# cornell-zhang/HiSparse

Hardware: AMD Instinct MI355X
Metric: SpMV GBPS (8 B per non-zero per SpMV, sw/benchmark.cpp:312-346) (higher is better)
Workload: dtype u32 (Q8.24 fixed point, u64 row sums)

## Files before the change

hisparse_amd/csrc/hs_api.cpp:

```cpp
#include "hs_context.h"

#include <algorithm>
#include <cctype>
#include <cstdlib>
#include <cstring>
#include <mutex>
#include <new>

#include "gpu_tiles.h"

namespace {

thread_local std::string g_create_error;

const char* const kOptionKeys[] = {
    "STREAM_FORMAT", "COL_SLICES", "MAX_ROWS", "CROSS_PARTITIONS", "SPMM_VECTORS", "ROW_RUNS", "AUX_BITS", "XCD_AFFINITY", "STREAM_RESIDENT", "RETILE", "PLAN_DEBUG",
    "BITMAP_SKEW", "BITMAP_X_LDS", "BITMAP_BUILD", "WALK_LANES", "NO_MFMA_IMAGE", "MFMA_CHUNK", "LIGHT", "LIGHT_WGS", "SWEEP",
    "DELTA_DEAL", "POW2_SLICES", "SPMM_FUSED", "SPMM_MFMA", "SPMSPV", "SPMSPV_CROSSOVER", "ITERATE_GRAPH", "BATCH_GRAPH", "CARRY_COMBINE", "AUTOTUNE", "PLAN_CENSUS",
    "VALUE_MAP",
};

hisparse::dev::SpmvLaunch launch_args(const hs_context* c, const uint32_t* x, uint32_t* y, int32_t filter) {
    hisparse::dev::SpmvLaunch a = c->mat.launch;
    a.x = x;
    a.out = c->mat.col_slices > 1 ? c->carry.partial() : y;
    a.row_part_filter = filter;
    return a;
}

void partition_rows(const hs_context* c, uint32_t j, uint32_t& lo, uint32_t& hi) {
    const uint64_t a = uint64_t(j) * c->geom.logical_ob;
    const uint64_t b = std::min<uint64_t>(a + c->geom.logical_ob, c->mat.num_rows);
    lo = uint32_t(a);
    hi = uint32_t(b);
}

int step(hs_context* c, int32_t filter = -1, const Feedback* feedback = nullptr) { return enqueue(c, c->x_source(), c->y_target(), filter, nullptr, nullptr, feedback); }

}

int fail(hs_context* ctx, int code, const std::string& msg) {
    if (ctx) ctx->error = msg; else g_create_error = msg;
    return code;
}
int hip_fail(hs_context* ctx, hipError_t e, const char* what) {
    return fail(ctx, HS_ERR_HIP, std::string(what) + ": " + hipGetErrorString(e));
}

int settle(hs_context* c) {
    const hipError_t e = c->carry.settle(c->stream);
    return e == hipSuccess ? HS_OK : hip_fail(c, e, "combine_slices_kernel");
}

int enter(hs_context* ctx, unsigned need) {
    if (!ctx) return HS_ERR_BAD_ARG;
    if ((need & kMatrix) && !ctx->mat.loaded) return fail(ctx, HS_ERR_NOT_LOADED, "hs_load_matrix has not been called");
    if (need & kVector) {
        if (!ctx->vector_loaded && !ctx->x_bound) return fail(ctx, HS_ERR_NOT_LOADED, "hs_load_vector has not been called");
        if (!ctx->x_bound && ctx->x_len != ctx->mat.num_cols)
            return fail(ctx, HS_ERR_NOT_LOADED, "the loaded vector does not have this matrix's padded column count: call hs_load_vector again");
    }
    if ((need & kCsc) && !ctx->csc.indptr) return fail(ctx, HS_ERR_NOT_LOADED, "hs_load_matrix_csc has not been called");
    if ((need & kHostOnly) == kHostOnly) return HS_OK;
    HS_HIP(ctx, hipSetDevice(ctx->device));
    return (need & kNoSettle) ? HS_OK : settle(ctx);
}
int enter(hs_context* ctx, unsigned need, bool have_args) {
    if (!ctx || !have_args) return fail(ctx, HS_ERR_BAD_ARG, "null argument");
    return enter(ctx, need);
}

void drop_batch_graph(hs_context* c) {
    if (c->batch_exec) (void)hipGraphExecDestroy(c->batch_exec);
    if (c->batch_graph) (void)hipGraphDestroy(c->batch_graph);
    c->batch_exec = nullptr;
    c->batch_graph = nullptr;
    c->batch_steps = 0;
}

// ... 55 lines not shown
    int rc = HS_OK;
    for (int i = 0; i < warm && rc == HS_OK; ++i) rc = enqueue(c, x, y, -1, nullptr, nullptr);
    for (int rep = 0; rep < regions && rc == HS_OK; ++rep) {
        (void)hipEventRecord(t0.get(), c->stream);
        for (int i = 0; i < runs && rc == HS_OK; ++i) rc = enqueue(c, x, y, -1, nullptr, nullptr);
        if (rc == HS_OK) rc = settle(c);
        (void)hipEventRecord(t1.get(), c->stream);
        float ms = 0.0f;
        if (rc == HS_OK && hipEventSynchronize(t1.get()) == hipSuccess && hipEventElapsedTime(&ms, t0.get(), t1.get()) == hipSuccess) {
            const double one = double(ms) * 1000.0 / runs;
            *us = *us < 0.0 ? one : std::min(*us, one);
        }
    }
    if (rc != HS_OK) {
        c->carry.forget();
        *us = -1.0;
    }
    return rc;
}

extern "C" {

const char* hs_strerror(int code) {
    switch (code) {
        case HS_OK: return "ok";
        case HS_ERR_BAD_ARG: return "bad argument";
        case HS_ERR_NO_DEVICE: return "no usable gfx950 device";
        case HS_ERR_HIP: return "HIP runtime error";
        case HS_ERR_BAD_MATRIX: return "channel buffers are not a valid CPSR image";
        case HS_ERR_NOT_LOADED: return "matrix or vector not loaded";
        case HS_ERR_UNSUPPORTED: return "unsupported configuration";
        case HS_ERR_NO_MEMORY: return "out of memory";
        default: return "unknown error";
    }
}

const char* hs_last_error(const hs_context* ctx) { return ctx ? ctx->error.c_str() : g_create_error.c_str(); }

int hs_create(hs_context** out, int device_id, int impl, uint32_t ob_bank, uint32_t vb_bank) {
    if (!out) return fail(nullptr, HS_ERR_BAD_ARG, "null context pointer");
    *out = nullptr;
    if (!hisparse::impl_valid(impl)) return fail(nullptr, HS_ERR_BAD_ARG, "impl must be 0 (fixed), 1 (float_pob) or 2 (float_stall)");
    int count = 0;
    hipError_t e = hipGetDeviceCount(&count);
    if (e != hipSuccess || count <= 0) return fail(nullptr, HS_ERR_NO_DEVICE, "no HIP device visible (this library has no CPU fallback)");
    if (device_id < 0 || device_id >= count) return fail(nullptr, HS_ERR_BAD_ARG, "device_id out of range");
    hipDeviceProp_t prop;
    if ((e = hipGetDeviceProperties(&prop, device_id)) != hipSuccess) return hip_fail(nullptr, e, "hipGetDeviceProperties");
    if (std::strncmp(prop.gcnArchName, "gfx950", 6) != 0)
        return fail(nullptr, HS_ERR_NO_DEVICE, std::string("device is ") + prop.gcnArchName + ", this library carries gfx950 code only");
    hs_context* c = new (std::nothrow) hs_context;
    if (!c) return fail(nullptr, HS_ERR_NO_MEMORY, "out of memory");
    c->device = device_id;
    c->impl = impl;
    c->geom = hisparse::make_geometry(impl, ob_bank ? ob_bank : hisparse::impl_default_ob_bank(impl),
                                      vb_bank ? vb_bank : hisparse::impl_default_vb_bank(impl));
    c->compute_units = prop.multiProcessorCount;
    if (c->geom.logical_ob > 0xffffffffull || c->geom.logical_vb > 0xffffffffull || c->geom.logical_ob % c->geom.row_divisor != 0) {
        delete c;
        return fail(nullptr, HS_ERR_BAD_ARG, "ob_bank must make 128*ob_bank a multiple of 128*interleave; bank sizes must fit 32 bits");
    }
    if ((e = hipSetDevice(device_id)) != hipSuccess || (e = hipStreamCreateWithFlags(&c->own_stream, hipStreamNonBlocking)) != hipSuccess) {
        delete c;
        return hip_fail(nullptr, e, "hipSetDevice/hipStreamCreate");
    }
    c->stream = c->own_stream;
    if ((e = hisparse::dev::configure_spmv_kernels(hisparse::dev::kMaxLdsBytes)) != hipSuccess || (e = hisparse::dev::warm_gpu_tiler()) != hipSuccess) {
        (void)hipStreamDestroy(c->own_stream);
        delete c;
        return hip_fail(nullptr, e, "loading the gfx950 kernels");
    }
    static std::once_flag copy_paths;
    std::call_once(copy_paths, [c] {
        std::vector<uint8_t> host(4 << 20, 0);
        DeviceBuffer<uint8_t> dev;
        if (dev.alloc(host.size()) != hipSuccess) return;
        (void)hipMemcpy(dev.get(), host.data(), host.size(), hipMemcpyHostToDevice);
        (void)hipMemcpy(host.data(), dev.get(), host.size(), hipMemcpyDeviceToHost);
        (void)hipMemcpyAsync(dev.get(), host.data(), host.size(), hipMemcpyHostToDevice, c->own_stream);
        (void)hipMemcpyAsync(host.data(), dev.get(), host.size(), hipMemcpyDeviceToHost, c->own_stream);
        (void)hipStreamSynchronize(c->own_stream);
    });
    *out = c;
    return HS_OK;
}

int hs_destroy(hs_context* ctx) {
    if (!ctx) return HS_OK;
    (void)hipSetDevice(ctx->device);
    if (ctx->stream == ctx->own_stream) (void)hipStreamSynchronize(ctx->own_stream);
    else (void)hipDeviceSynchronize();
    free_matrix(ctx);
    ctx->csc = CscData();
    ctx->d_x.reset();
    if (ctx->own_stream) (void)hipStreamDestroy(ctx->own_stream);
    delete ctx;
    return HS_OK;
}

int hs_load_vector(hs_context* ctx, const void* packed_x, uint32_t num_cols) {
    if (!ctx || !packed_x) return fail(ctx, HS_ERR_BAD_ARG, "null argument");
    if (ctx->mat.loaded && num_cols != ctx->mat.num_cols) return fail(ctx, HS_ERR_BAD_ARG, "vector length must equal the padded column count");
    if (int rc = enter(ctx, kNoSettle)) return rc;
    if (num_cols > ctx->x_capacity) {
        HS_HIP(ctx, hipStreamSynchronize(ctx->stream));
        ctx->x_capacity = 0;
        HS_HIP(ctx, ctx->d_x.alloc(size_t(num_cols) * 4 + 64));
        ctx->x_capacity = num_cols;
    }
    HS_HIP(ctx, hipMemcpyAsync(ctx->d_x.get(), packed_x, size_t(num_cols) * 4, hipMemcpyHostToDevice, ctx->stream));
    HS_HIP(ctx, hipStreamSynchronize(ctx->stream));
    ctx->vector_loaded = true;
    ctx->x_len = num_cols;
    return HS_OK;
}

int hs_run(hs_context* ctx) {
    if (int rc = enter(ctx, kReady | kNoSettle)) return rc;
    return step(ctx);
}

int hs_run_batch(hs_context* ctx, uint32_t steps) {
    int rc = enter(ctx, kReady | kNoSettle | (steps ? 0u : kHostOnly));
    if (rc != HS_OK || steps == 0) return rc;
    const char* opt = ctx_option(ctx, "HISPARSE_BATCH_GRAPH");
    struct InBatch {
        hs_context* c;
        const bool own;
        explicit InBatch(hs_context* ctx) : c(ctx), own(ctx->stream_private()) { c->in_batch = true; }
        ~InBatch() { c->in_batch = false; }
        int settle() { return own ? HS_OK : ::settle(c); }
    } batch(ctx);
    if (!(opt && std::atoi(opt) != 0)) {
        for (uint32_t i = 0; i < steps; ++i)
            if ((rc = step(ctx)) != HS_OK) {
                (void)batch.settle();
                return rc;
            }
        return batch.settle();
    }
    if (const char* why = hisparse::dev::profiling_switch_error()) return fail(ctx, HS_ERR_BAD_ARG, why);
    if (!ctx->batch_exec || ctx->batch_steps != steps || ctx->batch_x != ctx->x_source() || ctx->batch_y != ctx->y_target() || ctx->batch_stream != ctx->stream) {
        drop_batch_graph(ctx);
        if ((rc = ::settle(ctx)) != HS_OK) return rc;
        hipError_t e = hipStreamBeginCapture(ctx->stream, hipStreamCaptureModeThreadLocal);
        if (e != hipSuccess) return hip_fail(ctx, e, "hipStreamBeginCapture (the legacy default stream cannot be captured)");
        for (uint32_t i = 0; i < steps && rc == HS_OK; ++i) rc = step(ctx);
        if (rc == HS_OK) rc = ::settle(ctx);
        e = hipStreamEndCapture(ctx->stream, &ctx->batch_graph);
        if (rc == HS_OK && (e != hipSuccess || !ctx->batch_graph)) rc = hip_fail(ctx, e, "hipStreamEndCapture");
        if (rc == HS_OK && (e = hipGraphInstantiate(&ctx->batch_exec, ctx->batch_graph, nullptr, nullptr, 0)) != hipSuccess) rc = hip_fail(ctx, e, "hipGraphInstantiate");
        if (rc != HS_OK) {
            ctx->carry.forget();
            drop_batch_graph(ctx);
            return rc;
        }
        ctx->batch_steps = steps;
        ctx->batch_x = ctx->x_source();
        ctx->batch_y = ctx->y_target();
        ctx->batch_stream = ctx->stream;
    }
    if ((rc = ::settle(ctx)) != HS_OK) return rc;
    HS_HIP(ctx, hipGraphLaunch(ctx->batch_exec, ctx->stream));
    return HS_OK;
}

int hs_run_partition(hs_context* ctx, uint32_t row_part_id, uint32_t part_len) {
    if (int rc = enter(ctx, kReady | kNoSettle)) return rc;
    if (row_part_id >= ctx->mat.row_parts) return fail(ctx, HS_ERR_BAD_ARG, "row_part_id out of range");
    uint32_t lo, hi;
    partition_rows(ctx, row_part_id, lo, hi);
    if (part_len != (hi - lo) / hisparse::NUM_HBM_CHANNELS)
        return fail(ctx, HS_ERR_BAD_ARG, "part_len must be the partition's rows / 16 (sw/benchmark.cpp:301-322): expected " +
                                             std::to_string((hi - lo) / hisparse::NUM_HBM_CHANNELS));
    return step(ctx, int32_t(row_part_id));
}

int hs_feedback(hs_context* ctx, uint32_t scale_word, uint32_t shift_word) {
    if (int rc = enter(ctx, kReady)) return rc;
    HS_HIP(ctx, hisparse::dev::launch_feedback(ctx->is_float(), ctx->y_target(), const_cast<uint32_t*>(ctx->x_source()),
                                               std::min(ctx->mat.num_rows, ctx->mat.num_cols), scale_word, shift_word, ctx->stream));
    return HS_OK;
}

int hs_iterate(hs_context* ctx, uint32_t iterations, uint32_t scale_word, uint32_t shift_word) {
    int rc = enter(ctx, kReady | (iterations ? 0u : kHostOnly));
    if (rc != HS_OK || iterations == 0) return rc;
    const Feedback feedback{scale_word, shift_word};
    auto one_iteration = [&]() -> int { return step(ctx, -1, &feedback); };
    const char* graph_env = ctx_option(ctx, "HISPARSE_ITERATE_GRAPH");
    const bool use_graph = graph_env && std::atoi(graph_env) != 0;
    const uint32_t chunk = use_graph ? std::min<uint32_t>(iterations, 32) : 1;
    uint32_t done = 0;
    hipGraph_t graph = nullptr;
    hipGraphExec_t exec = nullptr;
    if (chunk > 1 && hipStreamBeginCapture(ctx->stream, hipStreamCaptureModeThreadLocal) == hipSuccess) {
        for (uint32_t i = 0; i < chunk && rc == HS_OK; ++i) rc = one_iteration();
        const hipError_t end = hipStreamEndCapture(ctx->stream, &graph);
        if (rc == HS_OK && end == hipSuccess && graph && hipGraphInstantiate(&exec, graph, nullptr, nullptr, 0) == hipSuccess) {
            hipError_t e = hipSuccess;
            for (; done + chunk <= iterations && e == hipSuccess; done += chunk) e = hipGraphLaunch(exec, ctx->stream);
            (void)hipGraphExecDestroy(exec);
            (void)hipGraphDestroy(graph);
            if (e != hipSuccess) return fail(ctx, HS_ERR_HIP, std::string("hipGraphLaunch: ") + hipGetErrorString(e));
        } else {
            if (graph) (void)hipGraphDestroy(graph);
            (void)hipGetLastError();
            if (rc != HS_OK) return rc;
        }
    } else {
        (void)hipGetLastError();
    }
    for (; done < iterations; ++done)
        if ((rc = one_iteration()) != HS_OK) return rc;
    return HS_OK;
}

int hs_sync(hs_context* ctx) {
    if (int rc = enter(ctx, 0)) return rc;
    HS_HIP(ctx, hipStreamSynchronize(ctx->stream));
    return HS_OK;
}

int hs_read_result(hs_context* ctx, void* packed_y, uint32_t num_rows) {
    if (int rc = enter(ctx, kMatrix | kNoSettle, packed_y != nullptr)) return rc;
    if (num_rows != ctx->mat.num_rows) return fail(ctx, HS_ERR_BAD_ARG, "result length must equal the padded row count");
    if (int rc = settle(ctx)) return rc;
    HS_HIP(ctx, hipMemcpyAsync(packed_y, ctx->y_target(), size_t(num_rows) * 4, hipMemcpyDeviceToHost, ctx->stream));
    HS_HIP(ctx, hipStreamSynchronize(ctx->stream));
    return HS_OK;
}

int hs_set_option(hs_context* ctx, const char* key, const char* value) {
    if (int rc = enter(ctx, kHostOnly, key != nullptr)) return rc;
    std::string k(key);
    for (char& ch : k) ch = char(std::toupper(static_cast<unsigned char>(ch)));
    if (k.rfind("HISPARSE_", 0) == 0) k = k.substr(9);
    bool known = false;
    for (const char* name : kOptionKeys) known = known || k == name;
    if (k == "ABLATE" || k == "DEPTH" || k == "TIMELINE_OUT")
        return fail(ctx, HS_ERR_BAD_ARG, "'" + k + "' is a profiling switch of libhisparse_hip_prof.so (wrong results by design), not an option of this library");
    if (!known) return fail(ctx, HS_ERR_BAD_ARG, "unknown option '" + std::string(key) + "'");
    if (value && *value && k == "MFMA_CHUNK") {
        uint32_t chunk = 0;
        if (!hisparse::dev::detail::parse_mfma_chunk(value, chunk)) return fail(ctx, HS_ERR_BAD_ARG, hisparse::dev::detail::kBadMfmaChunk);
    }
    if (value && *value) ctx->options["HISPARSE_" + k] = value;
    else ctx->options.erase("HISPARSE_" + k);
    drop_batch_graph(ctx);
    return HS_OK;
}

int hs_set_stream(hs_context* ctx, void* hip_stream) {
    if (int rc = enter(ctx, 0)) return rc;
// ... 52 lines not shown
    if (num_words > ctx->mat.num_rows || (num_words & 3u)) return fail(ctx, HS_ERR_BAD_ARG, "num_words must be a multiple of 4 and at most the padded row count");
    for (uint32_t k = 0; k < n_dst; ++k)
        if (!dst[k] || (reinterpret_cast<uintptr_t>(dst[k]) & 15u)) return fail(ctx, HS_ERR_BAD_ARG, "destinations must be 16-byte aligned device pointers");
    if (int rc = enter(ctx, 0)) return rc;
    HS_HIP(ctx, hisparse::dev::launch_push_result(ctx->y_target(), dst, n_dst, num_words, ctx->stream));
    return HS_OK;
}

int hs_get_stats(const hs_context* ctx, hs_stats* stats) {
    if (!ctx || !stats) return HS_ERR_BAD_ARG;
    *stats = ctx->stats;
    return HS_OK;
}

int hs_time_runs(hs_context* ctx, int warmup, int runs, float* total_ms, float* kernel_ms) {
    int rc = enter(ctx, kReady | kNoSettle);
    if (rc != HS_OK) return rc;
    if (warmup < 0 || runs <= 0) return fail(ctx, HS_ERR_BAD_ARG, "need warmup >= 0 and runs > 0");
    for (int i = 0; i < warmup; ++i)
        if ((rc = step(ctx)) != HS_OK) return rc;
    if ((rc = settle(ctx)) != HS_OK) return rc;
    HS_HIP(ctx, hipStreamSynchronize(ctx->stream));
    std::vector<DeviceEvent> events(2 + (kernel_ms ? size_t(runs) * 2 : 0));
    for (DeviceEvent& ev : events) HS_HIP(ctx, ev.create());
    const hipEvent_t begin = events[0].get(), end = events[1].get();
    const DeviceEvent* k = events.data() + 2;
    HS_HIP(ctx, hipEventRecord(begin, ctx->stream));
    for (int i = 0; i < runs; ++i)
        if ((rc = enqueue(ctx, ctx->x_source(), ctx->y_target(), -1, kernel_ms ? k[size_t(i) * 2].get() : nullptr, kernel_ms ? k[size_t(i) * 2 + 1].get() : nullptr)) != HS_OK) return rc;
    if ((rc = settle(ctx)) != HS_OK) return rc;
    HS_HIP(ctx, hipEventRecord(end, ctx->stream));
    HS_HIP(ctx, hipEventSynchronize(end));
    float ms = 0.0f;
    HS_HIP(ctx, hipEventElapsedTime(&ms, begin, end));
    if (total_ms) *total_ms = ms;
    if (kernel_ms) {
        float sum = 0.0f;
        for (int i = 0; i < runs; ++i) {
            float one = 0.0f;
            HS_HIP(ctx, hipEventElapsedTime(&one, k[size_t(i) * 2].get(), k[size_t(i) * 2 + 1].get()));
            sum += one;
        }
        *kernel_ms = sum;
    }
    return HS_OK;
}

int hs_time_kernel(hs_context* ctx, int warmup, int runs, float* kernel_ms) {
    int rc = enter(ctx, kReady | kHostOnly);
    if (rc != HS_OK) return rc;
    if (warmup < 0 || runs <= 0 || !kernel_ms) return fail(ctx, HS_ERR_BAD_ARG, "need warmup >= 0, runs > 0 and an output pointer");
    if (const char* why = hisparse::dev::profiling_switch_error()) return fail(ctx, HS_ERR_BAD_ARG, why);
    if ((rc = enter(ctx, 0)) != HS_OK) return rc;
    const hisparse::dev::SpmvLaunch args = launch_args(ctx, ctx->x_source(), ctx->y_target(), -1);
    const bool carried = ctx->carry.carries() && ctx->stream_private();
    auto launch = [&]() -> int {
        if (carried) return step(ctx);
        HS_HIP(ctx, hisparse::dev::launch_spmv(ctx->is_float(), args, ctx->stream));
        return HS_OK;
    };
    for (int i = 0; i < warmup; ++i)
        if ((rc = launch()) != HS_OK) return rc;
    DeviceEvent ev[2];
    HS_HIP(ctx, ev[0].create());
    HS_HIP(ctx, ev[1].create());
    HS_HIP(ctx, hipEventRecord(ev[0].get(), ctx->stream));
    for (int i = 0; i < runs; ++i)
        if ((rc = launch()) != HS_OK) return rc;
    HS_HIP(ctx, hipEventRecord(ev[1].get(), ctx->stream));
    HS_HIP(ctx, hipEventSynchronize(ev[1].get()));
    HS_HIP(ctx, hipEventElapsedTime(kernel_ms, ev[0].get(), ev[1].get()));
    return carried ? settle(ctx) : step(ctx);
}

}
```

hisparse_amd/csrc/hs_context.h:

```cpp
#ifndef HISPARSE_HS_CONTEXT_H_
#define HISPARSE_HS_CONTEXT_H_

#include "hisparse_hip.h"

#include <hip/hip_runtime_api.h>

#include <cstddef>
#include <cstdint>
#include <string>
#include <utility>
#include <vector>

#include "device_buffer.h"
#include "hisparse/common.h"
#include "spmv_kernels.h"
#include "stream_tiles.h"
#include "tiles_common.h"

class CarriedCombine {
public:
    void reset() { *this = CarriedCombine(); }
    hipError_t reset(bool is_float, uint32_t num_rows, uint32_t num_cols, uint32_t col_slices, bool carries) {
        reset();
        if (col_slices <= 1) return hipSuccess;
        const hipError_t e = partial_.alloc(size_t(carries ? 2 : 1) * col_slices * num_rows * 4);
        if (e != hipSuccess) return e;
        is_float_ = is_float;
        rows_ = num_rows;
        cols_ = num_cols;
        slices_ = col_slices;
        carries_ = carries;
        return hipSuccess;
    }

    bool carries() const { return carries_; }
    uint32_t* partial() const { return partial_.get(); }

    bool eligible(bool plain_whole_step, bool stream_private, const uint32_t* x, const uint32_t* y) const {
        return carries_ && plain_whole_step && stream_private && !aliases(x, y) && !(owed_ >= 0 && aliases(x, owed_y_));
    }

    hipError_t step(hisparse::dev::SpmvLaunch& a, uint32_t* y, hipStream_t stream) {
        const uint32_t b = turn_++ & 1u;
        const size_t set = size_t(slices_) * rows_;
        a.out = partial_.get() + b * set;
        if (owed_ >= 0) {
            a.carry_partial = partial_.get() + size_t(owed_) * set;
            a.carry_y = owed_y_;
            a.carry_rows = rows_;
            a.carry_slices = slices_;
        }
        const hipError_t e = hisparse::dev::launch_spmv(is_float_, a, stream);
        if (e != hipSuccess) return e;
        owed_ = int(b);
        owed_y_ = y;
        return hipSuccess;
    }

    hipError_t settle(hipStream_t stream) {
        if (owed_ < 0) return hipSuccess;
        const uint32_t* partial = partial_.get() + size_t(owed_) * slices_ * rows_;
        owed_ = -1;
        return hisparse::dev::launch_combine_slices(is_float_, partial, owed_y_, rows_, slices_, 0, rows_, stream);
    }

    void forget() { owed_ = -1; }

private:
    bool aliases(const uint32_t* x, const uint32_t* y) const {
        if (!x || !y) return false;
        const uintptr_t x0 = reinterpret_cast<uintptr_t>(x), x1 = x0 + size_t(cols_) * 4, y0 = reinterpret_cast<uintptr_t>(y), y1 = y0 + size_t(rows_) * 4;
        return x0 < y1 && y0 < x1;
    }

    DeviceBuffer<uint32_t> partial_;
    bool is_float_ = false, carries_ = false;
    uint32_t rows_ = 0, cols_ = 0, slices_ = 1;
    int owed_ = -1;
    uint32_t* owed_y_ = nullptr;
    uint32_t turn_ = 0;
};

struct MatrixData {
    bool loaded = false;
    uint32_t num_rows = 0, num_cols = 0, row_parts = 0;
    DeviceBuffer<uint8_t> image;
    DeviceBuffer<hisparse::dev::Block> blocks;
    DeviceBuffer<hisparse::dev::Unit> units;
    DeviceBuffer<uint32_t> part_heads;
    hisparse::dev::SpmvLaunch launch{};
    uint32_t col_slices = 1;
    bool crossing_blocks = false;
    uint32_t max_block_rows = 0;
    DeviceBuffer<uint32_t> y;
    DeviceBuffer<uint32_t> partition_y;
    uint32_t spmm_vectors = 1;
    DeviceBuffer<uint32_t> spmm_x4, spmm_partial, spmm_y;
    DeviceBuffer<uint32_t> x_interleaved;
    struct Mfma {
        DeviceBuffer<uint32_t> words;
        hisparse::dev::MfmaImage info;
        DeviceBuffer<uint32_t> x;
        DeviceBuffer<float> partial;
        DeviceBuffer<uint32_t> flag;
        DeviceBuffer<uint32_t> value_map;
    } mfma;
    DeviceBuffer<uint32_t> value_map;
    uint64_t value_map_nnz = 0;
    DeviceBuffer<float> value_stage;
    std::string value_map_why = "no matrix has been loaded";
};

struct CscData {
    DeviceBuffer<uint32_t> indptr, rows, vals;
    DeviceBuffer<uint32_t> keys, products, bin_base, cursors, overflow;
    uint64_t capacity = 0;
    hisparse::dev::SpmspvScratch scratch() const {
        return {keys.get(), products.get(), bin_base.get(), cursors.get(), overflow.get(), capacity};
    }
    std::vector<uint32_t> col_len;
    DeviceBuffer<uint32_t> y;
    uint32_t y_words = 0;
    PinnedBuffer<hisparse::dev::hs_idx_val_dev> h_sx;
    hisparse::dev::hs_idx_val_dev* d_sx = nullptr;
    DeviceEvent sx_read[2];
    uint32_t sx_turn = 0;
    std::vector<uint8_t> sx_seen;
    uint32_t sx_capacity = 0;
    DeviceBuffer<uint32_t> x_dense;
    uint32_t num_rows = 0, num_cols = 0;
};

struct hs_context {
    hisparse::dev::detail::OptionMap options;
    int device = -1;
    int impl = 0;
    hisparse::Geometry geom;
    hipStream_t own_stream = nullptr;
    hipStream_t stream = nullptr;
    int compute_units = 0;
    bool in_batch = false;
    bool stream_shared = false;

    MatrixData mat;
    CarriedCombine carry;
    CscData csc;
    uint32_t mfma_call = 0;
    double dense_spmv_us = 0.0;
    uint64_t spmspv_dense_dispatches = 0;

    hipGraph_t batch_graph = nullptr;
    hipGraphExec_t batch_exec = nullptr;
    uint32_t batch_steps = 0;
    const void* batch_x = nullptr;
    void* batch_y = nullptr;
    hipStream_t batch_stream = nullptr;

    bool vector_loaded = false;
    DeviceBuffer<uint32_t> d_x;
    const uint32_t* x_bound = nullptr;
    uint32_t* y_bound = nullptr;
    uint32_t x_capacity = 0;
    uint32_t x_len = 0;

    hs_stats stats{};
    std::string error;

    bool is_float() const { return impl != HS_IMPL_FIXED; }
    bool stream_private() const { return stream == own_stream && !stream_shared; }
    uint32_t* y_target() const { return y_bound ? y_bound : mat.y.get(); }
    const uint32_t* x_source() const { return x_bound ? x_bound : d_x.get(); }
};

int fail(hs_context* ctx, int code, const std::string& msg);
int hip_fail(hs_context* ctx, hipError_t e, const char* what);
#define HS_HIP(ctx, call)                                       \
    do {                                                        \
        hipError_t e_ = (call);                                 \
        if (e_ != hipSuccess) return hip_fail(ctx, e_, #call);  \
    } while (0)

inline const char* ctx_option(const hs_context* c, const char* name) { return hisparse::dev::detail::option_lookup(&c->options, name); }

enum : unsigned { kMatrix = 1u, kVector = 2u, kReady = kMatrix | kVector, kCsc = 4u, kNoSettle = 8u, kHostOnly = 16u | kNoSettle };
int enter(hs_context* ctx, unsigned need);
int enter(hs_context* ctx, unsigned need, bool have_args);
int settle(hs_context* ctx);

struct Feedback { uint32_t scale, shift; };
int enqueue(hs_context* c, const uint32_t* x, uint32_t* y, int32_t filter, hipEvent_t k0, hipEvent_t k1, const Feedback* feedback = nullptr);
int run_steps(hs_context* c, const uint32_t* x, uint64_t ldx, uint32_t* y, uint64_t ldy, uint32_t steps);
int time_steps(hs_context* c, const uint32_t* x, uint32_t* y, int warm, int regions, int runs, double* us);

void drop_batch_graph(hs_context* c);
void free_matrix(hs_context* c);

#endif
```

hisparse_amd/csrc/hs_load.cpp:

```cpp
#include "hs_context.h"

#include <algorithm>
#include <chrono>
#include <cstdio>
#include <cstdlib>

#include "hisparse/channel_packets.h"

using hisparse::Geometry;
using hisparse::dev::Block;
using hisparse::dev::Unit;

namespace {

constexpr size_t kImageSlackBytes = 16384;

bool value_map_asked(const hs_context* c) {
    const char* v = ctx_option(c, "HISPARSE_VALUE_MAP");
    return v && std::atoi(v) != 0;
}

template <typename T>
hipError_t upload(DeviceBuffer<T>& dst, const void* src, size_t bytes, size_t slack) {
    const hipError_t e = dst.alloc(std::max<size_t>(bytes + slack, 256));
// ... 56 lines not shown
                spmv::io::CSRMatrix<float> mat;
                mat.num_rows = rows->num_rows;
                mat.num_cols = rows->num_cols;
                const uint64_t nnz = rows->indptr[rows->num_rows];
                mat.adj_indptr.assign(rows->indptr, rows->indptr + rows->num_rows + 1);
                mat.adj_indices.assign(rows->indices, rows->indices + nnz);
                mat.adj_data.assign(rows->values, rows->values + nnz);
                const hisparse::ChannelPackets packets = hisparse::format_matrix(mat, g, true);
                const void* chan[hisparse::NUM_HBM_CHANNELS];
                uint64_t count[hisparse::NUM_HBM_CHANNELS];
                for (uint32_t c = 0; c < hisparse::NUM_HBM_CHANNELS; ++c) { chan[c] = packets.channel[c].data(); count[c] = packets.channel[c].size(); }
                ok = packets.num_rows == num_rows && packets.num_cols == num_cols &&
                     hisparse::dev::build_stream_tiles(chan, count, g, num_rows, num_cols, num_row_partitions, num_col_partitions, uint32_t(ctx->compute_units), tiles, why);
            } else {
                why = "CSR column index outside the matrix";
            }
        }
        if (!ok && !csr && on_gpu && why.rfind("gpu re-tile:", 0) == 0) {
            start_over_on_host();
            on_gpu = false;
            ok = hisparse::dev::build_stream_tiles(channel, n_packets, g, num_rows, num_cols, num_row_partitions, num_col_partitions,
                                                   uint32_t(ctx->compute_units), tiles, why);
        }
        if (!ok) rc = fail(ctx, why == hisparse::dev::detail::kBadMfmaChunk ? HS_ERR_BAD_ARG : HS_ERR_BAD_MATRIX, why);
    } catch (const std::bad_alloc&) {
        rc = fail(ctx, HS_ERR_NO_MEMORY, "out of host memory while re-tiling the matrix");
    } catch (const std::exception& e) {
        rc = fail(ctx, HS_ERR_BAD_MATRIX, std::string("re-tiling the matrix failed: ") + e.what());
    } catch (...) {
        rc = fail(ctx, HS_ERR_BAD_MATRIX, "re-tiling the matrix failed");
    }
    const bool image_on_device = tiles.d_image != nullptr, mfma_on_device = tiles.mfma.d_words != nullptr;
    adopt_device_images();
    if (rc != HS_OK) return rc;
    const bool debug = ctx_option(ctx, "HISPARSE_PLAN_DEBUG") != nullptr;
    auto since = [&]() { return std::chrono::duration<double, std::milli>(std::chrono::steady_clock::now() - t0).count(); };
    if (debug) std::fprintf(stderr, "load: image built after %.1f ms\n", since());
    const uint32_t lds_bytes = tiles.format == hisparse::dev::kFormatSweep ? hisparse::dev::spmv_sweep_lds_bytes(tiles.max_block_rows, ctx->is_float())
                               : tiles.light ? hisparse::dev::spmv_light_lds_bytes(tiles.max_block_rows)
                                           : hisparse::dev::spmv_lds_bytes(tiles.max_block_rows, tiles.ring_buffers, tiles.format) +
                                                 tiles.bitmap_x_groups * hisparse::dev::kBitmapGroupCols * 4u;
    if (lds_bytes > hisparse::dev::kMaxLdsBytes) return fail(ctx, HS_ERR_UNSUPPORTED, "row block does not fit the LDS");

    HS_HIP(ctx, hisparse::dev::configure_spmv_kernels(hisparse::dev::kMaxLdsBytes));
    if (!image_on_device)
        HS_HIP(ctx, upload(m.image, tiles.image.data(), tiles.image.size(), kImageSlackBytes));
    HS_HIP(ctx, upload(m.blocks, tiles.blocks.data(), tiles.blocks.size() * sizeof(Block), 0));
    HS_HIP(ctx, upload(m.units, tiles.units.data(), tiles.units.size() * sizeof(Unit), 0));
    HS_HIP(ctx, upload(m.part_heads, tiles.part_heads.data(), tiles.part_heads.size() * sizeof(uint32_t), 0));
    HS_HIP(ctx, m.y.alloc(size_t(num_rows) * 4));
    HS_HIP(ctx, hipMemset(m.y.get(), 0, size_t(num_rows) * 4));
    const uint64_t image_bytes = image_on_device ? tiles.image_bytes : uint64_t(tiles.image.size());
    const char* resident_opt = ctx_option(ctx, "HISPARSE_STREAM_RESIDENT");
    m.launch.stream_resident = resident_opt ? std::atoi(resident_opt) != 0
                                     : hisparse::dev::plan_stream_resident(tiles.format, tiles.light, image_bytes, tiles.units.size(), tiles.blocks.size(), tiles.value_bits);
    const char* carry_opt = ctx_option(ctx, "HISPARSE_CARRY_COMBINE");
    const uint64_t carry_bytes = tiles.format == hisparse::dev::kFormatDelta && tiles.value_bits == 24
                                     ? image_bytes / hisparse::dev::kRecordBytes24 * hisparse::dev::kRecordBytes : image_bytes;
    const bool carries = tiles.col_slices > 1 && (carry_opt ? std::atoi(carry_opt) != 0 : hisparse::dev::plan_carries(tiles.format, carry_bytes));
    HS_HIP(ctx, ctx->carry.reset(ctx->is_float(), num_rows, num_cols, tiles.col_slices, carries));
    if (mfma_on_device || (tiles.mfma.words_bytes != 0 && !tiles.mfma.words.empty())) {
        const hisparse::dev::MfmaImage& mi = tiles.mfma;
        MatrixData::Mfma& mf = m.mfma;
        bool ok = mfma_on_device || upload(mf.words, mi.words.data(), mi.words.size(), 0) == hipSuccess;
        ok = ok && mf.x.alloc(hisparse::dev::spmm_mfma_x_words(mi.groups) * 4) == hipSuccess &&
             mf.partial.alloc(hisparse::dev::spmm_mfma_partial_words(mi.tiles, mi.chunks) * 4) == hipSuccess &&
             mf.flag.alloc(64) == hipSuccess && hipMemset(mf.flag.get(), 0, 64) == hipSuccess;
        if (ok) {
            mf.info = std::move(tiles.mfma);
            mf.info.words = {};
        } else {
            (void)hipGetLastError();
            mf = MatrixData::Mfma();
        }
    }
    if (m.value_map) {
        m.value_map_nnz = tiles.nnz;
        m.value_map_why.clear();
    } else if (!map_on) {
        m.value_map_why = "the value_map option was off when the matrix was loaded";
    } else if (!csr) {
        m.value_map_why = "the matrix came from hs_load_matrix (CPSR): only hs_load_matrix_csr and hs_load_matrix_csr_transposed keep a value map";
    } else if (!image_on_device) {
        m.value_map_why = "the image was built by the host builder (duplicate (row, column) entries, bitmap_build=host, or SWEEP chunks spanning more than 65535 "
                          "columns): it has no value map";
    } else {
        m.value_map_why = "the image is 16 GiB or larger: its word indices do not fit 32 bits";
    }
    if (debug) std::fprintf(stderr, "load: descriptors + result buffers on the device after %.1f ms\n", since());
    m.num_rows = num_rows;
    m.num_cols = num_cols;
    m.row_parts = num_row_partitions;
    m.col_slices = tiles.col_slices;
    m.spmm_vectors = tiles.spmm_vectors;
    if (tiles.spmm_vectors == 4) {
        const uint32_t need = hisparse::dev::spmm_sweep_lds_bytes(tiles.max_block_rows, ctx->is_float());
        if (need > hisparse::dev::kMaxLdsBytes) m.spmm_vectors = 1;
        else HS_HIP(ctx, hisparse::dev::configure_spmm_sweep_kernels(hisparse::dev::kMaxLdsBytes));
    }
    for (const Block& b : tiles.blocks) m.crossing_blocks = m.crossing_blocks || b.last_part != b.row_part;
    m.max_block_rows = tiles.max_block_rows;
    hisparse::dev::SpmvLaunch& a = m.launch;
    a.image = m.image.get();
    a.blocks = m.blocks.get();
    a.units = m.units.get();
    a.part_heads = m.part_heads.get();
    a.ring_buffers = tiles.ring_buffers;
    a.format = tiles.format;
    a.value_bits = tiles.value_bits;
    a.num_cols = num_cols;
    a.num_workgroups = tiles.num_workgroups;
    a.lds_bytes = lds_bytes;
    a.bitmap_x_groups = tiles.bitmap_x_groups;
    a.light = tiles.light;
    ctx->dense_spmv_us = 0.0;
    m.loaded = true;

    hs_stats& s = ctx->stats;
    s = hs_stats{};
    s.nnz = tiles.nnz;
    for (int c = 0; n_packets && c < HS_NUM_CHANNELS; ++c) s.cpsr_bytes += n_packets[c] * sizeof(hisparse::MatPkt);
    s.stream_bytes = tiles.image_bytes;
    s.stream_elements = tiles.elements;
    s.num_blocks = uint32_t(tiles.blocks.size());
    s.num_units = uint32_t(tiles.units.size());
    s.col_slices = tiles.col_slices;
    s.ring_buffers = tiles.ring_buffers;
    s.stream_format = tiles.format;
    s.num_workgroups = tiles.num_workgroups;
    s.lds_bytes = lds_bytes;
    s.num_compute_units = uint32_t(ctx->compute_units);
    s.load_seconds = std::chrono::duration<double>(std::chrono::steady_clock::now() - t0).count();
    s.retiled_on_gpu = image_on_device;
    s.light_kernel = tiles.light ? 1u : 0u;
    s.value_bits = tiles.value_bits;
    s.stream_resident = a.stream_resident && hisparse::dev::stream_policy_applies(tiles.format, tiles.light) ? 1u : 0u;
    return HS_OK;
}

double time_loaded_plan(hs_context* ctx, int runs) {
    DeviceBuffer<uint32_t> zero_x;
    if (zero_x.alloc(size_t(ctx->mat.num_cols) * 4 + 64) != hipSuccess) { (void)hipGetLastError(); return -1.0; }
    double us = -1.0;
    if (hipMemsetAsync(zero_x.get(), 0, size_t(ctx->mat.num_cols) * 4, ctx->stream) == hipSuccess)
        (void)time_steps(ctx, zero_x.get(), ctx->mat.y.get(), 3, 2, runs, &us);
    (void)hipStreamSynchronize(ctx->stream);
    return us;
}

int load_matrix_impl(hs_context* ctx, const void* const* channel, const uint64_t* n_packets, const hisparse::dev::CsrView* csr,
                     uint32_t num_rows, uint32_t num_cols, uint32_t num_row_partitions, uint32_t num_col_partitions) {
    const char* tune = ctx_option(ctx, "HISPARSE_AUTOTUNE");
    const bool tuning = tune && std::atoi(tune) != 0 && !ctx_option(ctx, "HISPARSE_STREAM_FORMAT");
    int rc = load_matrix_once(ctx, channel, n_packets, csr, num_rows, num_cols, num_row_partitions, num_col_partitions, !tuning);
    if (rc != HS_OK || !tuning) return rc;
    const bool debug = ctx_option(ctx, "HISPARSE_PLAN_DEBUG") != nullptr;
    const char* const names[] = {"pairs", "delta", "bitmap", "owner", "pairs24", "owner24", "sweep"};
    const MatrixData& m = ctx->mat;
    const std::string own = m.launch.light ? "light" : names[m.launch.format < 7 ? m.launch.format : 0];
    const uint64_t nnz = ctx->stats.nnz;
    const int runs = int(std::max<uint64_t>(5, std::min<uint64_t>(50, (uint64_t(40) << 20) / std::max<uint64_t>(1, nnz))));
    double best_us = time_loaded_plan(ctx, runs);
    if (best_us <= 0.0)
        return value_map_asked(ctx) ? load_matrix_once(ctx, channel, n_packets, csr, num_rows, num_cols, num_row_partitions, num_col_partitions, true) : HS_OK;
    std::string best = own;
    if (debug) std::fprintf(stderr, "autotune: planner's plan %s x%u: %.2f us\n", own.c_str(), m.col_slices, best_us);
    const double own_us = best_us;
    const auto light_it = ctx->options.find("HISPARSE_LIGHT");
    const bool had_light = light_it != ctx->options.end();
    const std::string caller_light = had_light ? light_it->second : std::string();
    auto restore = [&]() {
        ctx->options.erase("HISPARSE_STREAM_FORMAT");
        if (had_light) ctx->options["HISPARSE_LIGHT"] = caller_light; else ctx->options.erase("HISPARSE_LIGHT");
    };
    for (const char* fmt : {"delta", "pairs", "owner24", "sweep"}) {
        if (own == fmt) continue;
        ctx->options["HISPARSE_STREAM_FORMAT"] = fmt;
        ctx->options["HISPARSE_LIGHT"] = "0";
        const int rc2 = load_matrix_once(ctx, channel, n_packets, csr, num_rows, num_cols, num_row_partitions, num_col_partitions, false);
        double us = -1.0;
        if (rc2 == HS_OK && std::string(names[m.launch.format < 7 ? m.launch.format : 0]) == fmt) us = time_loaded_plan(ctx, runs);
        if (debug) std::fprintf(stderr, "autotune: %s x%u: %s\n", fmt, rc2 == HS_OK ? m.col_slices : 0u, us > 0.0 ? (std::to_string(us) + " us").c_str() : "not available");
        if (us > 0.0 && us < 0.97 * best_us) { best_us = us; best = fmt; }
    }
    restore();
    if (best != own) {
        ctx->options["HISPARSE_STREAM_FORMAT"] = best;
        ctx->options["HISPARSE_LIGHT"] = "0";
    }
    rc = load_matrix_once(ctx, channel, n_packets, csr, num_rows, num_cols, num_row_partitions, num_col_partitions, true);
    restore();
    if (debug) std::fprintf(stderr, "autotune: kept %s (%.2f us against the planner's %.2f)\n", best.c_str(), best_us, own_us);
    return rc;
}

int update_values(hs_context* ctx, const float* values, uint64_t nnz, bool from_host) {
    if (int rc = enter(ctx, kMatrix | kHostOnly)) return rc;
    MatrixData& m = ctx->mat;
    if (!values) return fail(ctx, HS_ERR_BAD_ARG, "null argument");
    if (!m.value_map) return fail(ctx, HS_ERR_UNSUPPORTED, "no value map: " + m.value_map_why);
    if (nnz != m.value_map_nnz)
        return fail(ctx, HS_ERR_BAD_ARG, "nnz must equal the loaded CSR's indptr[num_rows] (" + std::to_string(m.value_map_nnz) + ")");
    if (!from_host && reinterpret_cast<uintptr_t>(values) % 4 != 0) return fail(ctx, HS_ERR_BAD_ARG, "values_dev must be 4-byte aligned");
    if (int rc = enter(ctx, 0)) return rc;
    if (nnz == 0) return HS_OK;
    const float* src = values;
    if (from_host) {
        if (!m.value_stage) HS_HIP(ctx, m.value_stage.alloc(size_t(nnz) * 4));
        HS_HIP(ctx, hipMemcpyAsync(m.value_stage.get(), values, size_t(nnz) * 4, hipMemcpyHostToDevice, ctx->stream));
        src = m.value_stage.get();
    }
    HS_HIP(ctx, hisparse::dev::launch_value_update(ctx->impl == HS_IMPL_FIXED, src, nnz, m.value_map.get(), reinterpret_cast<uint32_t*>(m.image.get()),
                                                   ctx->stats.stream_bytes / 4, m.mfma.value_map.get(), m.mfma.words.get(), m.mfma.value_map ? m.mfma.info.words_bytes / 4 : 0,
                                                   uint32_t(ctx->compute_units), ctx->stream));
    if (from_host) HS_HIP(ctx, hipStreamSynchronize(ctx->stream));
    return HS_OK;
}

int load_csr(hs_context* ctx, uint32_t num_rows, uint32_t num_cols, const uint32_t* indptr, const uint32_t* indices, const float* values, bool transposed,
             uint32_t* padded_rows, uint32_t* padded_cols) {
    if (!ctx || !indptr) return fail(ctx, HS_ERR_BAD_ARG, "null argument");
    const Geometry& g = ctx->geom;
    if (num_rows == 0 || num_cols == 0) return fail(ctx, HS_ERR_BAD_ARG, "empty matrix");
    hisparse::dev::CsrView view;
    view.num_rows = num_rows;
    view.num_cols = num_cols;
    view.indptr = indptr;
    view.indices = indices;
    view.values = values;
    view.transposed = transposed;
    const uint64_t rows = (uint64_t(view.out_rows()) + g.row_divisor - 1) / g.row_divisor * g.row_divisor;
    const uint64_t cols = (uint64_t(view.out_cols()) + hisparse::PACK_SIZE - 1) / hisparse::PACK_SIZE * hisparse::PACK_SIZE;
    if (rows > 0xffffffffull || cols > 0xffffffffull) return fail(ctx, HS_ERR_BAD_ARG, "padded dimensions exceed 32 bits");
    const int rc = load_matrix_impl(ctx, nullptr, nullptr, &view, uint32_t(rows), uint32_t(cols), uint32_t((rows + g.logical_ob - 1) / g.logical_ob),
                                    uint32_t((cols + g.logical_vb - 1) / g.logical_vb));
    if (rc == HS_OK) {
        if (padded_rows) *padded_rows = uint32_t(rows);
        if (padded_cols) *padded_cols = uint32_t(cols);
    }
    return rc;
}

}

extern "C" {

int hs_load_matrix(hs_context* ctx, const void* const channel[HS_NUM_CHANNELS], const uint64_t n_packets[HS_NUM_CHANNELS],
                   uint32_t num_rows, uint32_t num_cols, uint32_t num_row_partitions, uint32_t num_col_partitions) {
    if (!ctx || !channel || !n_packets) return fail(ctx, HS_ERR_BAD_ARG, "null argument");
    return load_matrix_impl(ctx, channel, n_packets, nullptr, num_rows, num_cols, num_row_partitions, num_col_partitions);
}

int hs_load_matrix_csr(hs_context* ctx, uint32_t num_rows, uint32_t num_cols, const uint32_t* indptr, const uint32_t* indices, const float* values,
                       uint32_t* padded_rows, uint32_t* padded_cols) {
    return load_csr(ctx, num_rows, num_cols, indptr, indices, values, false, padded_rows, padded_cols);
}

int hs_load_matrix_csr_transposed(hs_context* ctx, uint32_t num_rows, uint32_t num_cols, const uint32_t* indptr, const uint32_t* indices, const float* values,
                                  uint32_t* padded_rows, uint32_t* padded_cols) {
    return load_csr(ctx, num_rows, num_cols, indptr, indices, values, true, padded_rows, padded_cols);
}

int hs_update_values(hs_context* ctx, const float* values, uint64_t nnz) { return update_values(ctx, values, nnz, true); }
int hs_update_values_device(hs_context* ctx, const float* values_dev, uint64_t nnz) { return update_values(ctx, values_dev, nnz, false); }

int hs_debug_read_tiles(hs_context* ctx, void* image, uint64_t image_capacity, void* blocks, void* units) {
    if (int rc = enter(ctx, kMatrix | kHostOnly)) return rc;
// ... 24 lines not shown
```

hisparse_amd/csrc/stream_tiles.h:

```cpp
#ifndef HISPARSE_STREAM_TILES_H_
#define HISPARSE_STREAM_TILES_H_

#include <cstdint>
#include <string>
#include <memory>
#include <utility>
#include <vector>

#include "hisparse/common.h"

namespace hisparse {
namespace dev {

constexpr uint32_t kWaveLanes = 64;
constexpr uint32_t kWavesPerWorkgroup = 16;
constexpr uint32_t kConsumerWaves = 14;
constexpr uint32_t kLoaderWaves = kWavesPerWorkgroup - kConsumerWaves;
constexpr uint32_t kSubTileCols = 8192;
constexpr uint32_t kMaxXBuffers = 4;
constexpr uint32_t kMinXBuffers = 2;
constexpr uint32_t kAccumulatorBytes = 8;
constexpr uint32_t max_block_rows(bool sliced) { return (sliced ? 96u : 32u) * 1024u / kAccumulatorBytes - 1u; }
constexpr uint32_t kMaxColSlices = 8;
constexpr uint32_t kMaxForcedColSlices = 16;
constexpr uint32_t kMaxSweepSlices = 16;
constexpr uint64_t kCarryMaxImageBytes = 160ull << 20;
constexpr uint64_t kSlicedDeltaMaxImageBytes = 48ull << 20;
constexpr uint64_t kResidentMaxImageBytes = 256ull << 20;
constexpr uint64_t kRowblockResidentMaxImageBytes = 256ull << 20;
constexpr uint64_t kRowblockResidentSmallImageBytes = 32ull << 20;
constexpr uint32_t kMaxLdsBytes = 160 * 1024;
constexpr uint32_t kChunkBytes = kWaveLanes * 8;
constexpr uint32_t kWaveStrideBytes = kChunkBytes * kConsumerWaves;
constexpr uint32_t kRecordBytes = kWaveLanes * 2 * (4 + 2);
constexpr uint32_t kRecordBytes24 = kWaveLanes * (3 + 3 + 2 + 2);
constexpr uint32_t kMaxValueShift = 8;
constexpr uint64_t kDelta24OutlierShare = 4096;
constexpr uint64_t kDelta24MinSavedBytes = 23u << 20;
constexpr uint32_t delta_record_bytes(uint32_t value_bits) { return value_bits == 24 ? kRecordBytes24 : kRecordBytes; }
constexpr bool value_fits24(uint32_t word, uint32_t shift) { return (word >> shift) < (1u << 24) && (word & ((1u << shift) - 1u)) == 0; }
struct Outlier { uint32_t row, col, value; };
enum class DeltaValueBits : uint32_t { kByRule = 0, kPacked = 24, kPlain = 32 };
constexpr uint32_t kMaxGap = 0xfffeu;
constexpr uint32_t kBridgeGap = 0xffffu;
constexpr uint32_t kBridgeAdvance = 0xffffu;
constexpr double kDeltaMinMeanGap = 8.0;
constexpr double kDeltaMaxMeanGap = 20000.0;
constexpr uint64_t kDeltaMinSavedBytes = 23u << 20;
constexpr uint64_t kDeltaMinSavedBytesFloat = 40u << 20;
constexpr double kDenseMeanGap = 320.0;
enum StreamFormat : uint32_t { kFormatPairs = 0, kFormatDelta = 1, kFormatBitmap = 2, kFormatOwner = 3, kFormatPairs24 = 4, kFormatOwner24 = 5, kFormatSweep = 6 };
constexpr bool rowblock_stream(uint32_t format, bool light) { return (format == kFormatPairs || format == kFormatDelta) && !light; }
constexpr bool stream_policy_applies(uint32_t format, bool light) { return format == kFormatSweep || rowblock_stream(format, light); }
constexpr bool plan_stream_resident(uint32_t format, bool light, uint64_t image_bytes, uint64_t num_units, uint64_t num_blocks, uint32_t value_bits = 0) {
    const uint64_t judged_bytes = format == kFormatDelta && value_bits == 24 ? image_bytes / kRecordBytes24 * kRecordBytes : image_bytes;
    return rowblock_stream(format, light)
               ? judged_bytes <= kRowblockResidentMaxImageBytes && (num_units > num_blocks || judged_bytes <= kRowblockResidentSmallImageBytes)
               : image_bytes <= kResidentMaxImageBytes;
}
constexpr bool plan_carries(uint32_t format, uint64_t image_bytes) {
    return image_bytes < kCarryMaxImageBytes || format == kFormatOwner || format == kFormatOwner24;
}
constexpr uint32_t kChunkBytes24 = kWaveLanes * 7;
constexpr uint32_t kWaveStrideBytes24 = kChunkBytes24 * kConsumerWaves;
constexpr uint32_t kAux24MaxRows = 2046;
constexpr uint32_t kOwnerRecordSteps = 4;
constexpr uint32_t kOwnerRecordValueBytes = kWaveLanes * 4 * kOwnerRecordSteps;
constexpr uint32_t kOwnerRecordBytes = kOwnerRecordValueBytes + kWaveLanes * 3 * kOwnerRecordSteps;
constexpr uint32_t kOwnerSpareField = 2047;
constexpr uint32_t kOwnerShareRows = 2047;
constexpr uint32_t kOwnerStepMask = 0xffffu;
constexpr uint32_t kOwnerAccumulatorBytes = 4;
constexpr uint32_t kOwnerColBits = 13;
constexpr uint32_t owner_max_block_rows(uint32_t ring) { return (kMaxLdsBytes - ring * kSubTileCols * 4u) / kOwnerAccumulatorBytes - kConsumerWaves - 1u; }
constexpr double kOwnerMinMeanGap = 20000.0;
constexpr double kBitmapMinDensity = 0.125;
constexpr uint32_t kBitmapMinCols = 2048;
constexpr uint32_t kBitmapGroupCols = 64;
#ifndef HS_BITMAP_WAVES
#define HS_BITMAP_WAVES 16
#endif
constexpr uint32_t kBitmapWaves = HS_BITMAP_WAVES;
constexpr uint32_t kBitmapMaxBlockRows = 8191;
constexpr uint32_t kBitmapMaxXLdsGroups = 576;
constexpr uint32_t kBitmapSkew[4] = {170, 140, 65, 25};
constexpr uint32_t kBitmapMaskBatch = 32;
constexpr uint32_t kBitmapRunSlots = 5;
constexpr uint64_t kLightMaxNnz = 2u << 20;
constexpr uint32_t kLightMaxUnits = 16;
constexpr uint32_t kLightWorkgroupsPerCu = 4;
constexpr uint32_t kLightMaxBlockRows = 3071;
constexpr uint32_t kLightMinBlockNnz = 1024;
#ifndef HS_SWEEP_WAVES
#define HS_SWEEP_WAVES 8
#endif
constexpr uint32_t kSweepWaves = HS_SWEEP_WAVES;
constexpr uint32_t kSweepMaxBlockRowsFloat = kMaxLdsBytes / kAccumulatorBytes - 1;
constexpr uint32_t kSweepMaxBlockRowsFixed = (kMaxLdsBytes / 4 - 2) * 32 / 33 - 1;
constexpr uint32_t kSweepColAlign = 32;
constexpr double kSweepSlabMinMeanGap = 8000.0;
constexpr uint64_t kSweepMinNnz = (2u << 20) + 1;
constexpr uint64_t kFloatOneSliceOwnerMinNnz = 8u << 20;
constexpr uint64_t kSweepMinNnzWide = 256u << 10;
constexpr uint32_t kDenseBlockRows = 32;
constexpr uint32_t kBlockDenseRows = 1u;
constexpr uint32_t kBlockLastOfPartition = 2u;
constexpr uint32_t kNoBlock = 0xffffffffu;

struct Block {
    uint32_t row0;
// ... 109 lines not shown
```

Before: 6579.

## Track cache reuse of matrix images per device to gate resident streaming per launch

Adds a per-device LRU reuse tracker that records which matrix images were launched recently and their byte sizes. Each launch now chooses the stream-resident (cache-retaining) load policy only when the image is eligible and is still estimated to be warm in the last-level cache. Graph capture and replay paths snapshot and touch the tracker. The delta-24 size adjustment in the eligibility test is dropped, and the first launch of any image now runs non-resident. This may lower throughput when the estimate is wrong or when only one matrix is ever used.

```diff
diff --git a/hisparse_amd/csrc/hs_api.cpp b/hisparse_amd/csrc/hs_api.cpp
--- a/hisparse_amd/csrc/hs_api.cpp
+++ b/hisparse_amd/csrc/hs_api.cpp
@@ -20,11 +20,36 @@
     "VALUE_MAP",
 };
 
-hisparse::dev::SpmvLaunch launch_args(const hs_context* c, const uint32_t* x, uint32_t* y, int32_t filter) {
+static_assert(hisparse::dev::kRowblockResidentMaxImageBytes == hisparse::dev::kResidentMaxImageBytes, "one cache, one budget for the reuse tracker");
+
+bool launch_stream_resident(hs_context* c) {
+    const MatrixData& m = c->mat;
+    const uint64_t budget = hisparse::dev::kResidentMaxImageBytes;
+    if (c->capturing) return hisparse::launch_resident(c->capture_list, m.resident_forced, m.resident_eligible, m.image_id, m.image_bytes, budget);
+    hipStreamCaptureStatus capture = hipStreamCaptureStatusNone;
+    if (c->stream != c->own_stream && hipStreamIsCapturing(c->stream, &capture) == hipSuccess && capture != hipStreamCaptureStatusNone) {
+        hisparse::ReuseList copy = c->reuse->snapshot();
+        return hisparse::launch_resident(copy, m.resident_forced, m.resident_eligible, m.image_id, m.image_bytes, budget);
+    }
+    return c->reuse->launch_resident(m.resident_forced, m.resident_eligible, m.image_id, m.image_bytes, budget);
+}
+
+struct CaptureScope {
+    hs_context* c;
+    explicit CaptureScope(hs_context* ctx) : c(ctx) {
+        c->capture_list = c->reuse->snapshot();
+        c->capturing = true;
+    }
+    ~CaptureScope() { c->capturing = false; }
+};
+void replayed(hs_context* c) { c->reuse->touch(c->mat.image_id, c->mat.image_bytes); }
+
+hisparse::dev::SpmvLaunch launch_args(hs_context* c, const uint32_t* x, uint32_t* y, int32_t filter) {
     hisparse::dev::SpmvLaunch a = c->mat.launch;
     a.x = x;
     a.out = c->mat.col_slices > 1 ? c->carry.partial() : y;
     a.row_part_filter = filter;
+    a.stream_resident = launch_stream_resident(c);
     return a;
 }
 
@@ -186,6 +211,7 @@
     hs_context* c = new (std::nothrow) hs_context;
     if (!c) return fail(nullptr, HS_ERR_NO_MEMORY, "out of memory");
     c->device = device_id;
+    c->reuse = &hisparse::reuse_tracker_for(device_id);
     c->impl = impl;
     c->geom = hisparse::make_geometry(impl, ob_bank ? ob_bank : hisparse::impl_default_ob_bank(impl),
                                       vb_bank ? vb_bank : hisparse::impl_default_vb_bank(impl));
@@ -279,7 +305,10 @@
         if ((rc = ::settle(ctx)) != HS_OK) return rc;
         hipError_t e = hipStreamBeginCapture(ctx->stream, hipStreamCaptureModeThreadLocal);
         if (e != hipSuccess) return hip_fail(ctx, e, "hipStreamBeginCapture (the legacy default stream cannot be captured)");
-        for (uint32_t i = 0; i < steps && rc == HS_OK; ++i) rc = step(ctx);
+        {
+            CaptureScope capture(ctx);
+            for (uint32_t i = 0; i < steps && rc == HS_OK; ++i) rc = step(ctx);
+        }
         if (rc == HS_OK) rc = ::settle(ctx);
         e = hipStreamEndCapture(ctx->stream, &ctx->batch_graph);
         if (rc == HS_OK && (e != hipSuccess || !ctx->batch_graph)) rc = hip_fail(ctx, e, "hipStreamEndCapture");
@@ -296,6 +325,7 @@
     }
     if ((rc = ::settle(ctx)) != HS_OK) return rc;
     HS_HIP(ctx, hipGraphLaunch(ctx->batch_exec, ctx->stream));
+    replayed(ctx);
     return HS_OK;
 }
 
@@ -329,11 +359,17 @@
     hipGraph_t graph = nullptr;
     hipGraphExec_t exec = nullptr;
     if (chunk > 1 && hipStreamBeginCapture(ctx->stream, hipStreamCaptureModeThreadLocal) == hipSuccess) {
-        for (uint32_t i = 0; i < chunk && rc == HS_OK; ++i) rc = one_iteration();
+        {
+            CaptureScope capture(ctx);
+            for (uint32_t i = 0; i < chunk && rc == HS_OK; ++i) rc = one_iteration();
+        }
         const hipError_t end = hipStreamEndCapture(ctx->stream, &graph);
         if (rc == HS_OK && end == hipSuccess && graph && hipGraphInstantiate(&exec, graph, nullptr, nullptr, 0) == hipSuccess) {
             hipError_t e = hipSuccess;
-            for (; done + chunk <= iterations && e == hipSuccess; done += chunk) e = hipGraphLaunch(exec, ctx->stream);
+            for (; done + chunk <= iterations && e == hipSuccess; done += chunk) {
+                e = hipGraphLaunch(exec, ctx->stream);
+                replayed(ctx);
+            }
             (void)hipGraphExecDestroy(exec);
             (void)hipGraphDestroy(graph);
             if (e != hipSuccess) return fail(ctx, HS_ERR_HIP, std::string("hipGraphLaunch: ") + hipGetErrorString(e));
@@ -492,10 +528,10 @@
     if (warmup < 0 || runs <= 0 || !kernel_ms) return fail(ctx, HS_ERR_BAD_ARG, "need warmup >= 0, runs > 0 and an output pointer");
     if (const char* why = hisparse::dev::profiling_switch_error()) return fail(ctx, HS_ERR_BAD_ARG, why);
     if ((rc = enter(ctx, 0)) != HS_OK) return rc;
-    const hisparse::dev::SpmvLaunch args = launch_args(ctx, ctx->x_source(), ctx->y_target(), -1);
     const bool carried = ctx->carry.carries() && ctx->stream_private();
     auto launch = [&]() -> int {
         if (carried) return step(ctx);
+        const hisparse::dev::SpmvLaunch args = launch_args(ctx, ctx->x_source(), ctx->y_target(), -1);
         HS_HIP(ctx, hisparse::dev::launch_spmv(ctx->is_float(), args, ctx->stream));
         return HS_OK;
     };
diff --git a/hisparse_amd/csrc/hs_context.h b/hisparse_amd/csrc/hs_context.h
--- a/hisparse_amd/csrc/hs_context.h
+++ b/hisparse_amd/csrc/hs_context.h
@@ -13,6 +13,7 @@
 
 #include "device_buffer.h"
 #include "hisparse/common.h"
+#include "reuse_tracker.h"
 #include "spmv_kernels.h"
 #include "stream_tiles.h"
 #include "tiles_common.h"
@@ -89,6 +90,9 @@
     DeviceBuffer<hisparse::dev::Unit> units;
     DeviceBuffer<uint32_t> part_heads;
     hisparse::dev::SpmvLaunch launch{};
+    uint64_t image_id = 0, image_bytes = 0;
+    int resident_forced = -1;
+    bool resident_eligible = false;
     uint32_t col_slices = 1;
     bool crossing_blocks = false;
     uint32_t max_block_rows = 0;
@@ -156,6 +160,10 @@
     void* batch_y = nullptr;
     hipStream_t batch_stream = nullptr;
 
+    hisparse::ReuseTracker* reuse = nullptr;
+    hisparse::ReuseList capture_list;
+    bool capturing = false;
+
     bool vector_loaded = false;
     DeviceBuffer<uint32_t> d_x;
     const uint32_t* x_bound = nullptr;
diff --git a/hisparse_amd/csrc/hs_load.cpp b/hisparse_amd/csrc/hs_load.cpp
--- a/hisparse_amd/csrc/hs_load.cpp
+++ b/hisparse_amd/csrc/hs_load.cpp
@@ -132,8 +132,11 @@
     HS_HIP(ctx, hipMemset(m.y.get(), 0, size_t(num_rows) * 4));
     const uint64_t image_bytes = image_on_device ? tiles.image_bytes : uint64_t(tiles.image.size());
     const char* resident_opt = ctx_option(ctx, "HISPARSE_STREAM_RESIDENT");
-    m.launch.stream_resident = resident_opt ? std::atoi(resident_opt) != 0
-                                     : hisparse::dev::plan_stream_resident(tiles.format, tiles.light, image_bytes, tiles.units.size(), tiles.blocks.size(), tiles.value_bits);
+    m.resident_forced = resident_opt ? int(std::atoi(resident_opt) != 0) : -1;
+    m.resident_eligible = hisparse::dev::stream_policy_applies(tiles.format, tiles.light) &&
+                          hisparse::dev::plan_stream_resident(tiles.format, tiles.light, image_bytes, tiles.units.size(), tiles.blocks.size());
+    m.image_id = hisparse::next_image_id();
+    m.image_bytes = image_bytes;
     const char* carry_opt = ctx_option(ctx, "HISPARSE_CARRY_COMBINE");
     const uint64_t carry_bytes = tiles.format == hisparse::dev::kFormatDelta && tiles.value_bits == 24
                                      ? image_bytes / hisparse::dev::kRecordBytes24 * hisparse::dev::kRecordBytes : image_bytes;
@@ -214,7 +217,7 @@
     s.retiled_on_gpu = image_on_device;
     s.light_kernel = tiles.light ? 1u : 0u;
     s.value_bits = tiles.value_bits;
-    s.stream_resident = a.stream_resident && hisparse::dev::stream_policy_applies(tiles.format, tiles.light) ? 1u : 0u;
+    s.stream_resident = (m.resident_forced >= 0 ? m.resident_forced != 0 : m.resident_eligible) && hisparse::dev::stream_policy_applies(tiles.format, tiles.light) ? 1u : 0u;
     return HS_OK;
 }
 
@@ -293,6 +296,7 @@
     HS_HIP(ctx, hisparse::dev::launch_value_update(ctx->impl == HS_IMPL_FIXED, src, nnz, m.value_map.get(), reinterpret_cast<uint32_t*>(m.image.get()),
                                                    ctx->stats.stream_bytes / 4, m.mfma.value_map.get(), m.mfma.words.get(), m.mfma.value_map ? m.mfma.info.words_bytes / 4 : 0,
                                                    uint32_t(ctx->compute_units), ctx->stream));
+    m.image_id = hisparse::next_image_id();
     if (from_host) HS_HIP(ctx, hipStreamSynchronize(ctx->stream));
     return HS_OK;
 }
diff --git a/hisparse_amd/csrc/reuse_tracker.h b/hisparse_amd/csrc/reuse_tracker.h
--- /dev/null
+++ b/hisparse_amd/csrc/reuse_tracker.h
@@ -0,0 +1,79 @@
+#ifndef HISPARSE_REUSE_TRACKER_H_
+#define HISPARSE_REUSE_TRACKER_H_
+
+#include <atomic>
+#include <cstdint>
+#include <memory>
+#include <mutex>
+#include <vector>
+
+namespace hisparse {
+
+constexpr uint32_t kReuseListEntries = 32;
+
+struct ReuseList {
+    struct Entry { uint64_t id, bytes; };
+    Entry entry[kReuseListEntries] = {};
+    uint32_t count = 0;
+
+    bool touch(uint64_t id, uint64_t bytes, uint64_t budget) {
+        uint32_t at = 0;
+        uint64_t distance = bytes;
+        bool sums = true;
+        while (at < count && entry[at].id != id) {
+            sums = sums && distance + entry[at].bytes >= distance;
+            distance += entry[at].bytes;
+            ++at;
+        }
+        const bool warm = at < count && sums && distance <= budget;
+        if (at == count && count < kReuseListEntries) ++count;
+        if (at == kReuseListEntries) --at;
+        for (; at > 0; --at) entry[at] = entry[at - 1];
+        entry[0] = Entry{id, bytes};
+        return warm;
+    }
+};
+
+inline bool launch_resident(ReuseList& list, int forced, bool eligible, uint64_t id, uint64_t bytes, uint64_t budget) {
+    const bool warm = list.touch(id, bytes, budget);
+    return forced >= 0 ? forced != 0 : eligible && warm;
+}
+
+class ReuseTracker {
+public:
+    bool launch_resident(int forced, bool eligible, uint64_t id, uint64_t bytes, uint64_t budget) {
+        std::lock_guard<std::mutex> hold(lock_);
+        return hisparse::launch_resident(list_, forced, eligible, id, bytes, budget);
+    }
+    void touch(uint64_t id, uint64_t bytes) {
+        std::lock_guard<std::mutex> hold(lock_);
+        (void)list_.touch(id, bytes, 0);
+    }
+    ReuseList snapshot() const {
+        std::lock_guard<std::mutex> hold(lock_);
+        return list_;
+    }
+
+private:
+    mutable std::mutex lock_;
+    ReuseList list_;
+};
+
+inline ReuseTracker& reuse_tracker_for(int device) {
+    static std::mutex lock;
+    static auto& trackers = *new std::vector<std::unique_ptr<ReuseTracker>>;
+    std::lock_guard<std::mutex> hold(lock);
+    const size_t at = device < 0 ? 0 : size_t(device);
+    if (trackers.size() <= at) trackers.resize(at + 1);
+    if (!trackers[at]) trackers[at].reset(new ReuseTracker);
+    return *trackers[at];
+}
+
+inline uint64_t next_image_id() {
+    static std::atomic<uint64_t> last{0};
+    return last.fetch_add(1, std::memory_order_relaxed) + 1;
+}
+
+}
+
+#endif
diff --git a/hisparse_amd/csrc/stream_tiles.h b/hisparse_amd/csrc/stream_tiles.h
--- a/hisparse_amd/csrc/stream_tiles.h
+++ b/hisparse_amd/csrc/stream_tiles.h
@@ -52,10 +52,9 @@
 enum StreamFormat : uint32_t { kFormatPairs = 0, kFormatDelta = 1, kFormatBitmap = 2, kFormatOwner = 3, kFormatPairs24 = 4, kFormatOwner24 = 5, kFormatSweep = 6 };
 constexpr bool rowblock_stream(uint32_t format, bool light) { return (format == kFormatPairs || format == kFormatDelta) && !light; }
 constexpr bool stream_policy_applies(uint32_t format, bool light) { return format == kFormatSweep || rowblock_stream(format, light); }
-constexpr bool plan_stream_resident(uint32_t format, bool light, uint64_t image_bytes, uint64_t num_units, uint64_t num_blocks, uint32_t value_bits = 0) {
-    const uint64_t judged_bytes = format == kFormatDelta && value_bits == 24 ? image_bytes / kRecordBytes24 * kRecordBytes : image_bytes;
+constexpr bool plan_stream_resident(uint32_t format, bool light, uint64_t image_bytes, uint64_t num_units, uint64_t num_blocks) {
     return rowblock_stream(format, light)
-               ? judged_bytes <= kRowblockResidentMaxImageBytes && (num_units > num_blocks || judged_bytes <= kRowblockResidentSmallImageBytes)
+               ? image_bytes <= kRowblockResidentMaxImageBytes && (num_units > num_blocks || image_bytes <= kRowblockResidentSmallImageBytes)
                : image_bytes <= kResidentMaxImageBytes;
 }
 constexpr bool plan_carries(uint32_t format, uint64_t image_bytes) {
```

Measured after the change: 7320 (median of 6 runs). 1.11x the previous value.
